# ad3002/aindex

Measured on AMD Instinct MI355X. Metric: kmer_lookups_per_sec_23mer_batch, higher is better.
Workload: dtype u64

## Files before the change

### aindex_amd/_lib.py

```python
from __future__ import annotations

import ctypes as C
import os
import re
import subprocess

_HERE = os.path.dirname(os.path.abspath(__file__))
ROOT = os.path.dirname(_HERE)
LIB_PATH = os.path.join(_HERE, "lib", "libaindex_hip.so")
CSRC = os.path.join(_HERE, "csrc")
HEADER = os.path.join(ROOT, "include", "aindex_hip.h")

AIX_OK = 0
AIX_ERR_CONFLICT = -12
AIX_ERR_ARG = -1
AIX_ERR_FORMAT = -3
AIX_ERR_NOMEM = -4
AIX_ERR_UNSUPPORTED = -6
AIX_ERR_MODE = -7
FMT_AUTO, FMT_PLAIN, FMT_FASTA, FMT_FASTQ = -1, 0, 1, 2
CANON_NONE, CANON_REF_X86, CANON_TRUE_RC = 0, 1, 2
TOTAL_13MERS = 4 ** 13
DIR_NEXT, DIR_PREV, DIR_BOTH = 0, 1, 2
WALK_GREEDY, WALK_UNITIG = 0, 1
# ... 27 lines not shown
                ("buckets", C.c_uint64), ("bucket_unfiled_keys", C.c_uint64), ("bucket_lanes", C.c_uint32), ("absence_filter_words", C.c_uint32),
                ("minimizer_lines", C.c_uint64), ("minimizer_unfiled_keys", C.c_uint64), ("count23_backend", C.c_uint32), ("count23_passes", C.c_uint32), ("positions_backend", C.c_uint32), ("reserved0", C.c_uint32),
                ("aindex_attached", C.c_uint32), ("ridx_on_device", C.c_uint32), ("aindex_entries", C.c_uint64), ("ridx_reads", C.c_uint64)]


class IngestStats(C.Structure):
    _fields_ = [("bytes_in", C.c_uint64), ("plain_bytes", C.c_uint64), ("parts", C.c_uint64), ("part_bytes", C.c_uint64), ("pieces", C.c_uint64),
                ("pinned_bytes", C.c_uint64), ("device_bytes", C.c_uint64), ("workspace_bytes", C.c_uint64), ("seconds_total", C.c_double), ("seconds_read", C.c_double),
                ("seconds_wait", C.c_double), ("seconds_h2d", C.c_double), ("seconds_normalise", C.c_double), ("seconds_compute", C.c_double), ("seconds_output", C.c_double)]

    def as_dict(self):
        return {n: getattr(self, n) for n, _ in self._fields_}


CONT_FIELDS = [("tf", "<u4", (4,)), ("n", "<u4"), ("sum", "<u4"), ("best_tf", "<u4"), ("best_base", "<u4")]


def cont_dtype():
    import numpy as np
    return np.dtype(CONT_FIELDS)


def readfix_dtype():
    import numpy as np
    return np.dtype(READFIX_FIELDS)


_LIB = None
vp, u64, u32, i32 = C.c_void_p, C.c_uint64, C.c_uint32, C.c_int

SIGNATURES = {
    "aix_version": (C.c_char_p, []),
    "aix_strerror": (C.c_char_p, [i32]),
    "aix_device_count": (i32, [C.POINTER(i32)]),
    "aix_pf_check": (i32, [vp, u64, C.POINTER(u64 * 4)]),
    "aix_index_open_23": (i32, [C.c_char_p, C.c_char_p, C.c_char_p, i32, C.POINTER(vp)]),
    "aix_index_open_13": (i32, [C.c_char_p, C.c_char_p, i32, C.POINTER(vp)]),
    "aix_index_create_23": (i32, [vp, u64, vp, vp, u64, i32, C.POINTER(vp)]),
    "aix_index_create_13": (i32, [vp, u64, vp, i32, C.POINTER(vp)]),
    "aix_index_close": (i32, [vp]),
    "aix_index_info": (i32, [vp, C.POINTER(Info)]),
    "aix_index_set_canonical_fastpath": (i32, [vp, i32]),
    "aix_index_set_fingerprint_filter": (i32, [vp, i32]),
    "aix_index_set_early_exit": (i32, [vp, i32]),
    "aix_index_set_bucket_table": (i32, [vp, i32, i32]),
    "aix_index_set_absence_filter": (i32, [vp, i32]),
    "aix_index_set_minimizer_table": (i32, [vp, i32]),
    "aix_index_set_tf_13": (i32, [vp, vp]),
    "aix_index_get_tf": (i32, [vp, vp, u64]),
    "aix_index_get_checker": (i32, [vp, vp, u64]),
    "aix_tf_batch_ascii": (i32, [vp, vp, u64, vp]),
    "aix_tf_batch_ascii_dev": (i32, [vp, vp, u64, vp, vp]),
    "aix_lookup_binned_stats": (i32, [vp, vp]),
    "aix_tf_batch_codes": (i32, [vp, vp, u64, vp]),
    "aix_tf_batch_codes_dev": (i32, [vp, vp, u64, vp, vp]),
    "aix_tf_batch_ragged": (i32, [vp, vp, vp, u64, vp]),
    "aix_tf_batch_ragged_dev": (i32, [vp, vp, vp, u64, vp, vp]),
    "aix_lines_batch_ascii_dev": (i32, [vp, vp, u64, vp, vp]),
    "aix_hash_batch_ascii": (i32, [vp, vp, u64, vp]),
    "aix_hash_batch_ascii_dev": (i32, [vp, vp, u64, vp, vp]),
    "aix_kid_strand_batch_ascii": (i32, [vp, vp, u64, vp, vp]),
    "aix_kid_strand_batch_ascii_dev": (i32, [vp, vp, u64, vp, vp, vp]),
    "aix_tf_both_batch_ascii": (i32, [vp, vp, u64, vp, vp]),
    "aix_tf_both_batch_ascii_dev": (i32, [vp, vp, u64, vp, vp, vp]),
    "aix_tf_total_batch_ascii": (i32, [vp, vp, u64, vp]),
    "aix_tf_total_batch_ascii_dev": (i32, [vp, vp, u64, vp, vp]),
    "aix_coverage_batch": (i32, [vp, vp, vp, u64, u32, vp, vp]),
    "aix_coverage_batch_dev": (i32, [vp, vp, vp, u64, u64, u32, vp, vp, vp]),
    "aix_count13": (i32, [vp, vp, u64, i32, vp]),
    "aix_count13_dev": (i32, [vp, vp, u64, vp, vp]),
    "aix_count23_fixed": (i32, [vp, vp, u64, i32, i32, vp]),
    "aix_count23_fixed_dev": (i32, [vp, vp, u64, i32, vp, vp]),
    "aix_ingest_warm": (i32, [i32]),
    "aix_count13_file": (i32, [vp, C.c_char_p, i32, C.c_char_p, vp, C.POINTER(IngestStats)]),
    "aix_count23_fixed_file": (i32, [vp, C.c_char_p, i32, i32, vp, C.POINTER(IngestStats)]),
    "aix_count_distinct_file": (i32, [C.c_char_p, i32, i32, i32, u64, i32, C.POINTER(vp), C.POINTER(vp), C.POINTER(u64), C.POINTER(IngestStats)]),
    "aix_merge_runs_dev": (i32, [vp, vp, vp, u32, u64, i32, vp, C.POINTER(vp)]),
    "aix_count_distinct": (i32, [vp, u64, i32, i32, i32, u64, i32, C.POINTER(vp), C.POINTER(vp), C.POINTER(u64)]),
    "aix_positions_fill": (i32, [vp, vp, u64, vp, vp, u64, C.POINTER(u64)]),
    "aix_positions_total": (i32, [vp, C.POINTER(u64)]),
    "aix_positions_fill_dev": (i32, [vp, vp, u64, u64, vp, vp, u64, vp]),
    "aix_positions_bucket_counts": (i32, [vp, vp, u64, i32, vp]),
    "aix_aindex_attach": (i32, [vp, vp, vp, u64]),
    "aix_aindex_attach_dev": (i32, [vp, vp, vp, u64, vp]),
    "aix_aindex_detach": (i32, [vp]),
    "aix_ridx_sorted_disjoint": (i32, [vp, u64]),
    "aix_ridx_attach": (i32, [vp, vp, u64]),
    "aix_positions_query": (i32, [vp, vp, u64, u64, C.POINTER(vp), C.POINTER(vp), C.POINTER(vp), C.POINTER(vp)]),
    "aix_positions_query_dev": (i32, [vp, vp, u64, u64, vp, vp, vp, vp, u64, C.POINTER(u64), vp]),
    "aix_positions_locate": (i32, [vp, vp, u64, vp, vp]),
    "aix_positions_locate_dev": (i32, [vp, vp, u64, vp, vp, vp]),
    "aix_reads_attach": (i32, [vp, vp, u64]),
    "aix_reads_attach_dev": (i32, [vp, vp, u64, vp]),
    "aix_reads_detach": (i32, [vp]),
    "aix_reads_info": (i32, [vp, C.POINTER(u64 * 2)]),
    "aix_reads_fetch": (i32, [vp, vp, vp, vp, u64, C.POINTER(vp), C.POINTER(vp)]),
    "aix_reads_fetch_dev": (i32, [vp, vp, vp, vp, u64, vp, vp, u64, C.POINTER(u64), vp]),
    "aix_reads_fetch_rid": (i32, [vp, vp, u64, C.POINTER(vp), C.POINTER(vp)]),
    "aix_reads_fetch_rid_dev": (i32, [vp, vp, u64, vp, vp, u64, C.POINTER(u64), vp]),
    "aix_reads_by_kmers": (i32, [vp, vp, u64, u64, C.POINTER(vp), C.POINTER(vp), C.POINTER(vp), C.POINTER(vp)]),
    "aix_reads_by_kmers_dev": (i32, [vp, vp, u64, u64, vp, vp, vp, u64, vp, u64, C.POINTER(u64 * 2), vp]),
    "aix_neighbours": (i32, [vp, vp, vp, u64, i32, u32, vp]),
    "aix_neighbours_dev": (i32, [vp, vp, vp, u64, i32, u32, vp, vp]),
    "aix_walk": (i32, [vp, vp, vp, u64, i32, u64, u32, i32, vp, vp, vp, vp, vp]),
    "aix_walk_dev": (i32, [vp, vp, vp, u64, i32, u64, u32, i32, vp, vp, vp, vp, vp, vp]),
    "aix_unitigs_layout_dev": (i32, [vp, u32, vp, vp, vp, C.POINTER(u64), C.POINTER(u64), C.POINTER(u64), C.POINTER(u64), vp]),
# ... 144 lines not shown
```

### aindex_amd/csrc/aix_device.hpp

```cpp
#pragma once
#include <hip/hip_runtime.h>
#include <stdint.h>

#define AIX_HD __host__ __device__ __forceinline__

namespace aix {

struct __attribute__((aligned(16))) BvRec {
    uint32_t pairs;
    uint32_t prefix;
    uint64_t fp;
};
struct __attribute__((aligned(32))) EeRec {
    uint32_t pairs;
    uint32_t prefix;
    uint32_t mask[6];
};
struct __attribute__((aligned(16))) KeyRec {
    uint64_t code;
    uint32_t tf;
    uint32_t pad;
};

struct __attribute__((aligned(16))) BkEntry {
    uint32_t code_lo;
    uint32_t code_hi;
    uint32_t tf;
    uint32_t slot;
};
#define AIX_BK_HI_MASK 0x3FFFFFFFu
#define AIX_BK_OVERFLOW 0x80000000u
#define AIX_BK_EMPTY_HI 0x3FFFFFFFu
#define AIX_BK_NONE 0xFFFFFFFFu

AIX_HD uint32_t rot32(uint32_t x, uint32_t k) { return (x << k) | (x >> (32u - k)); }
AIX_HD void filter_key(uint64_t code, uint32_t& hw, uint32_t& hb) {
    uint32_t a = (uint32_t)code + 0x9E3779B9u, b = (uint32_t)(code >> 32) + 0x85EBCA6Bu, c = 0xC2B2AE35u;
    c ^= b; c -= rot32(b, 14);
    a ^= c; a -= rot32(c, 11);
    b ^= a; b -= rot32(a, 25);
    c ^= b; c -= rot32(b, 16);
    a ^= c; a -= rot32(c, 4);
    b ^= a; b -= rot32(a, 14);
    c ^= b; c -= rot32(b, 24);
    hw = b;
    hb = c;
}
AIX_HD uint64_t bloom_mask(uint32_t hb) {
    const uint32_t lo = (1u << (hb & 15)) | (0x10000u << ((hb >> 4) & 15)), hi = (1u << ((hb >> 8) & 15)) | (0x10000u << ((hb >> 12) & 15));
    return (uint64_t)lo | ((uint64_t)hi << 32);
}
AIX_HD uint32_t bloom_word(uint32_t hw, uint32_t nwords) { return (uint32_t)(((uint64_t)hw * nwords) >> 32); }

struct FastMod {
    uint64_t d;
    uint32_t dn;
    uint32_t v;
    uint32_t s;
    uint32_t wide;
};

inline FastMod make_fastmod(uint64_t d) {
    FastMod f{};
    f.d = d;
    if (d == 0) { f.wide = 1; f.d = 1; return f; }
    if (d >> 32) { f.wide = 1; return f; }
    uint32_t d32 = (uint32_t)d;
    f.s = (uint32_t)__builtin_clz(d32);
    f.dn = d32 << f.s;
    f.v = (uint32_t)((~0ull) / f.dn - (1ull << 32));
    return f;
}

AIX_HD uint32_t rem_2by1(uint32_t u1, uint32_t u0, uint32_t d, uint32_t v) {
    uint64_t q = (uint64_t)v * u1 + (((uint64_t)u1 << 32) | u0);
    uint32_t q1 = (uint32_t)(q >> 32) + 1u, q0 = (uint32_t)q;
    uint32_t r = u0 - q1 * d;
    if (r > q0) r += d;
    if (r >= d) r -= d;
    return r;
}

AIX_HD uint64_t fastmod(uint64_t h, const FastMod& f) {
    if (f.wide) return h % f.d;
    const uint32_t s = f.s;
    const uint32_t hi = (uint32_t)(h >> 32), lo = (uint32_t)h;
    const uint32_t u2 = s ? (hi >> (32 - s)) : 0u;
    const uint32_t u1 = s ? ((hi << s) | (lo >> (32 - s))) : hi;
    const uint32_t u0 = lo << s;
    uint32_t r = rem_2by1(u2, u1, f.dn, f.v);
    r = rem_2by1(r, u0, f.dn, f.v);
    return (uint64_t)(r >> s);
}

AIX_HD void jmix(uint64_t& a, uint64_t& b, uint64_t& c) {
    a -= b; a -= c; a ^= (c >> 43);
    b -= c; b -= a; b ^= (a << 9);
    c -= a; c -= b; c ^= (b >> 8);
    a -= b; a -= c; a ^= (c >> 38);
    b -= c; b -= a; b ^= (a << 23);
    c -= a; c -= b; c ^= (b >> 5);
    a -= b; a -= c; a ^= (c >> 35);
    b -= c; b -= a; b ^= (a << 49);
    c -= a; c -= b; c ^= (b >> 11);
// ... 452 lines not shown
```

### aindex_amd/csrc/aix_handle.hpp

```cpp
#pragma once
#include <hip/hip_runtime.h>

#include <mutex>
#include <string>

#include "../../include/aindex_hip.h"
#include "aix_internal.hpp"

using namespace aix;

void set_last_error(const std::string& s);

#define HIPCHK(expr)                                                                          \
    do {                                                                                      \
        hipError_t _e = (expr);                                                               \
        if (_e != hipSuccess) {                                                               \
            set_last_error(std::string(#expr) + ": " + hipGetErrorString(_e));                \
            return AIX_ERR_HIP;                                                               \
        }                                                                                     \
    } while (0)


struct DevGuard {
    int prev = -1;
// ... 15 lines not shown
    bool pooled = true;
    hipError_t alloc(uint64_t bytes) { return pool_alloc(&p, bytes ? bytes : 1); }
    hipError_t alloc_once(uint64_t bytes) { pooled = false; return hipMalloc(&p, bytes ? bytes : 1); }
    ~DevBuf() { if (p) { (void)hipStreamSynchronize(st); if (pooled) pool_free(p); else (void)hipFree(p); } }
};

struct aix_index {
    int device = 0;
    uint32_t k = 0;
    uint64_t n = 0;
    uint64_t mphf_n = 0, D = 0, seed = 0, B = 0, W = 0;
    BvRec* recs = nullptr;
    EeRec* ee = nullptr;
    KeyRec* keys = nullptr;
    uint32_t* side = nullptr;
    KeyRec* unfiled = nullptr;
    uint64_t n_unfiled = 0;
    BkEntry* bk = nullptr;
    uint32_t nb = 0;
    bool bk_borrowed = false;
    uint32_t bk_lpp = 8;
    bool bk_lpp_set = false;
    uint64_t bk_unfiled = 0;
    bool bk_enabled = true;
    BkEntry* mk = nullptr;
    uint32_t* mk_off = nullptr;
    uint32_t mk_cap = 16;
    uint32_t nbm = 0;
    uint64_t mk_unfiled = 0;
    bool mk_enabled = true;
    uint64_t* bloom = nullptr;
    uint32_t nbloom = 0;
    bool bloom_enabled = true;
    uint64_t* tf13_mphf = nullptr;
    uint64_t* tf13_code = nullptr;
    uint32_t* perm13 = nullptr;
    unsigned long long* scratch13 = nullptr;
    void* count_ws = nullptr;
    uint64_t count_ws_bytes = 0;
    void* pin_in = nullptr;
    void* pin_out[3] = {nullptr, nullptr, nullptr};
    std::mutex small_mutex;
    hipStream_t small_stream = nullptr;
    void* pin_cov = nullptr;
    struct HostPipe* pipe = nullptr;
    std::mutex pipe_mutex;
    hipEvent_t count_done = nullptr;
    hipStream_t hist_stream = nullptr;
    hipStream_t probe_stream = nullptr;
    hipEvent_t probe_ev[2] = {nullptr, nullptr}, hist_ev[2] = {nullptr, nullptr}, start_ev = nullptr;
    void* lb_ws = nullptr;
    uint64_t lb_ws_bytes = 0;
    uint64_t* lb_stats = nullptr;
    hipEvent_t lb_done = nullptr;
    hipStream_t lb_stream = nullptr;
    bool lb_used = false;
    std::mutex lb_mutex;
    uint64_t device_bytes = 0;
    bool perm13_bijective = false;
    bool canonical_only = false;
    bool canonical_fastpath = true;
    bool has_fp = false;
    bool fp_filter = true;
    bool early_exit = true;
    std::mutex count_mutex;
    uint64_t pos_total = 0;
    bool pos_total_known = false;
    uint32_t a2_backend = 0;
    uint32_t c23_backend = 0, c23_passes = 0;
    bool c13_atomics = false, c13_added = false;
    uint64_t* ai_indices = nullptr;
    uint64_t* ai_positions = nullptr;
    uint64_t ai_total = 0;
    bool ai_attached = false, ai_owned = false;
    uint64_t* rx = nullptr;
    uint64_t rx_n = 0;
    bool rx_attached = false;
    uint8_t* rd = nullptr;
    uint64_t rd_len = 0;
    bool rd_attached = false, rd_owned = false;

    IndexDev dev_slots() const {
        IndexDev d = dev();
        if (!bk_lpp_set) d.bk_lpp = 2;
        return d;
    }
    IndexDev dev() const {
        IndexDev d{};
        d.m.recs = recs;
        d.m.ee = ee;
        d.m.D = D;
        d.m.seed = seed;
        d.m.nrecs = (B + 15) / 16;
        d.m.fm = make_fastmod(D);
        d.keys = keys;
        d.side = side;
        d.bk_store = bk;
        d.unfiled = unfiled;
        d.n = n;
        d.tf13_code = tf13_code;
        d.tf13_mphf = tf13_mphf;
        d.perm13 = perm13;
        d.canonical_only = (canonical_only && canonical_fastpath) ? 1u : 0u;
        d.k = k;
        d.use_fp = (has_fp && fp_filter) ? 1u : 0u;
        d.early_exit = (has_fp && ee && early_exit) ? 1u : 0u;
// ... 33 lines not shown
```

### aindex_amd/csrc/aix_lookup_binned.hip

```cpp
#include <algorithm>

#include "aix_env.hpp"
#include "aix_handle.hpp"

namespace aix {

static constexpr int LB_TB = 512;
static constexpr int LB_QPL = 8;
static constexpr int LB_TILE = LB_TB * LB_QPL;
static constexpr int LB_CH = 256;
static constexpr int LB_LINE = 16;
static constexpr int LB_MAXBINS = 256;
static_assert(LB_CH % LB_LINE == 0 && LB_LINE <= 64, "lines do not straddle chunks; one wave instruction moves a carry");
static constexpr unsigned LB_GRID_A = 768;
static constexpr int LB_FB = 512;
static constexpr int LB_CPG = LB_FB / LB_CH;
static constexpr int LB_U = 2;
static constexpr int LB_CPT = LB_U * LB_CPG;
static constexpr int LB_TICKETS = 8;
static constexpr int LB_SURV = 4096;
static constexpr int LB_FLUSH_AT = LB_SURV - LB_U * LB_FB;
static constexpr unsigned LB_GRID_B = 1024;
static_assert(LB_FB % LB_CH == 0 && LB_FB >= LB_MAXBINS && LB_FB % 64 == 0, "pass B scans the slices' chunk counts with one lane per slice");
static_assert(LB_FLUSH_AT > 0, "LB_SURV holds the flush threshold plus one trip's records");
static constexpr uint32_t LB_SAMPLES = 16384;
static constexpr uint32_t LB_IDX_BITS = 27, LB_WORD_BITS = 18, LB_MASK_BITS = 16;
static_assert(LB_MASK_BITS == 16 && LB_IDX_BITS + LB_WORD_BITS + LB_MASK_BITS <= 64, "the record holds the 16 bits bloom_mask reads");
static constexpr uint32_t LB_NONE = 0xFFFFFFFFu;
static constexpr uint32_t LB_LO_BITS = 32 - LB_IDX_BITS, LB_META_LO = 9;
static_assert(LB_IDX_BITS < 32 && LB_MAXBINS < (1 << LB_META_LO) && LB_META_LO + LB_LO_BITS <= 16 && LB_TILE <= (1 << 13), "that word never equals LB_NONE");
static constexpr uint64_t LB_HDR_BYTES = 4096;
enum { LB_FLAG = 0, LB_PASSED = 1, LB_DONE = 2, LB_NSURV = 3, LB_CURSOR = 16, LB_TICKET = 512 };

static constexpr uint32_t LB_NO_SHIFT = 32;
struct LbGeom {
    uint32_t nbins;
    uint32_t wps;
    uint32_t inv;
    uint32_t shift;
    uint32_t cap;
};
struct LbWs {
    uint32_t* hdr;
    uint32_t* list;
    uint32_t* cnt;
    uint64_t* rec;
    unsigned long long* stats;
};

__device__ __forceinline__ bool lb_hash(uint64_t w0, uint64_t w1, uint64_t w2, uint32_t& hw, uint32_t& hb) {
    uint64_t code;
    if (!encode23_clean(w0, w1, w2, code)) return false;
    const uint64_t r = revcomp(code, 23);
    filter_key(code <= r ? code : r, hw, hb);
    return true;
}

__device__ __forceinline__ void lb_slice(uint32_t word, const LbGeom& g, uint32_t& bin, uint32_t& wi) {
    if (g.shift != LB_NO_SHIFT) {
        bin = word >> g.shift;
        wi = word & (g.wps - 1);
    } else {
        bin = __umulhi(word, g.inv);
        wi = word - bin * g.wps;
        if (wi >= g.wps) { wi -= g.wps; ++bin; }
    }
}

__global__ void __launch_bounds__(256) k_lb_gate(const uint64_t* __restrict__ bloom, uint32_t nbloom, const uint8_t* __restrict__ q, uint32_t n,
                                                 uint32_t nsamp, int force, uint32_t* __restrict__ hdr, unsigned long long* __restrict__ stats) {
    if (force) {
        if (blockIdx.x == 0 && threadIdx.x == 0) { hdr[LB_FLAG] = 1u; atomicAdd(&stats[0], 1ull); }
        return;
    }
    __shared__ uint32_t s_pass;
    if (threadIdx.x == 0) s_pass = 0;
    __syncthreads();
    const uint32_t s = blockIdx.x * 256 + threadIdx.x;
    bool pass = false;
    if (s < nsamp) {
        const uint64_t i = (uint64_t)s * n / nsamp;
        uint64_t w0, w1, w2;
        uint32_t hw, hb;
        load23(q + 23 * i, w0, w1, w2);
// ... 228 lines not shown
        __syncthreads();
        for (uint32_t i = t; i < s_n; i += LB_FB) w.list[s_base + i] = surv[i];
        __syncthreads();
        if (t == 0) s_n = 0;
        __syncthreads();
    };
    const uint32_t nt = min(gridDim.x, (uint32_t)LB_TICKETS);
    const uint32_t lane_x = blockIdx.x % nt;
    uint32_t* const ticket = w.hdr + LB_TICKET + 32 * lane_x;
    uint32_t bin = 0;
    for (;;) {
        if (t == 0) s_ticket = atomicAdd(ticket, 1u);
        __syncthreads();
        const uint64_t it64 = ((uint64_t)s_ticket * nt + lane_x) * LB_CPT;
        if (it64 >= total) break;
        const uint32_t it = (uint32_t)it64;
        uint64_t r[LB_U], wd[LB_U];
        uint32_t cn[LB_U], wbase[LB_U];
#pragma unroll
        for (int u = 0; u < LB_U; ++u) {
            const uint32_t item = it + u * LB_CPG + t / LB_CH;
            cn[u] = 0; r[u] = 0; wbase[u] = 0;
            if (item < total) {
                while (bin + 1 < NB && item >= pre[bin + 1]) ++bin;
                const uint64_t ch = (uint64_t)bin * g.cap + (item - pre[bin]);
                cn[u] = w.cnt[ch];
                r[u] = __builtin_nontemporal_load(&w.rec[ch * LB_CH + t % LB_CH]);
                wbase[u] = bin * g.wps;
            }
        }
#pragma unroll
        for (int u = 0; u < LB_U; ++u) {
            const uint32_t word = wbase[u] + ((uint32_t)(r[u] >> LB_IDX_BITS) & ((1u << LB_WORD_BITS) - 1));
            wd[u] = (t % LB_CH < cn[u] && word < nbloom) ? bloom[word] : 0ull;
        }
#pragma unroll
        for (int u = 0; u < LB_U; ++u) {
            const uint64_t mk = bloom_mask((uint32_t)(r[u] >> (LB_IDX_BITS + LB_WORD_BITS)));
            const bool pass = t % LB_CH < cn[u] && (wd[u] & mk) == mk;
            const uint64_t m = __ballot(pass);
            if (m) {
                uint32_t r0 = 0;
                if ((t & 63u) == 0) r0 = atomicAdd(&s_n, (uint32_t)__popcll(m));
                r0 = __shfl(r0, 0);
                if (pass) surv[r0 + (uint32_t)__popcll(m & ((1ull << (t & 63u)) - 1))] = (uint32_t)r[u] & ((1u << LB_IDX_BITS) - 1);
            }
        }
        __syncthreads();
        if (s_n > (uint32_t)LB_FLUSH_AT) flush();
    }
    if (s_n) flush();
}

}

static uint64_t align_up(uint64_t x, uint64_t a) { return (x + a - 1) / a * a; }

void lookup_binned_release(aix_index* h) {
    if (h->lb_done) { (void)hipEventSynchronize(h->lb_done); (void)hipEventDestroy(h->lb_done); h->lb_done = nullptr; }
    if (h->lb_ws) { (void)hipFree(h->lb_ws); h->lb_ws = nullptr; h->lb_ws_bytes = 0; }
    if (h->lb_stats) { (void)hipFree(h->lb_stats); h->lb_stats = nullptr; }
}

int lookup23_binned(aix_index* h, const IndexDev& d, const uint8_t* q, uint64_t N, uint32_t* out, hipStream_t s) {
    const long sw = env_int("AIX_LOOKUP_BINNED", 0, 2, 1);
    if (sw == 0 || d.k != 23 || !d.canonical_only || !d.bk || !d.bloom || d.nbloom == 0) return AIX_LB_NOT_TAKEN;
    if (sw == 1 && N < env_u64("AIX_LOOKUP_BINNED_MIN", 0, ~0ull, AIX_LB_DEFAULT_MIN)) return AIX_LB_NOT_TAKEN;
    const uint64_t slice_bytes = env_u64("AIX_LOOKUP_SLICE_BYTES", 8, 2ull << 20, 1ull << 20);
    LbGeom g;
    g.wps = (uint32_t)std::min<uint64_t>(std::max<uint64_t>(slice_bytes / 8, 1), d.nbloom);
    g.nbins = (d.nbloom + g.wps - 1) / g.wps;
    if (g.nbins > (uint32_t)LB_MAXBINS) return AIX_LB_NOT_TAKEN;
    g.inv = g.wps > 1 ? (uint32_t)((1ull << 32) / g.wps) : 0xFFFFFFFFu;
    g.shift = (g.wps & (g.wps - 1)) == 0 ? (uint32_t)__builtin_ctz(g.wps) : LB_NO_SHIFT;
    const uint64_t piece = std::min<uint64_t>(std::min<uint64_t>(N, 1ull << LB_IDX_BITS), env_u64("AIX_LOOKUP_PIECE", 1, 1ull << LB_IDX_BITS, 1ull << LB_IDX_BITS));
    const uint64_t test_grid_a = env_u64("AIX_LOOKUP_TEST_GRID_A", 1, LB_GRID_A, LB_GRID_A);
    const unsigned grid_a = (unsigned)std::min<uint64_t>((piece + LB_TILE - 1) / LB_TILE, test_grid_a);
    const uint32_t carry_bytes = g.nbins * LB_LINE * 8;
    const uint64_t test_cap = env_u64("AIX_LOOKUP_TEST_BIN_CAP", 0, ~0ull, ~0ull);
    uint64_t cap = test_cap != ~0ull ? (test_cap + LB_CH - 1) / LB_CH : (piece + piece / 4) / g.nbins / LB_CH + 2 + grid_a;
    cap = std::min<uint64_t>(cap, (piece + LB_CH - 1) / LB_CH + grid_a);
    g.cap = (uint32_t)cap;
    const uint64_t off_list = LB_HDR_BYTES, off_cnt = align_up(off_list + 4 * piece, 256), off_rec = align_up(off_cnt + 4ull * g.nbins * cap, 256);
    const uint64_t need = off_rec + 8ull * g.nbins * cap * LB_CH;

    std::lock_guard<std::mutex> lk(h->lb_mutex);
    if (!h->lb_done && hipEventCreateWithFlags(&h->lb_done, hipEventDisableTiming) != hipSuccess) { (void)hipGetLastError(); h->lb_done = nullptr; return AIX_LB_NOT_TAKEN; }
    if (!h->lb_stats) {
        if (hipMalloc((void**)&h->lb_stats, 32) != hipSuccess) { (void)hipGetLastError(); h->lb_stats = nullptr; return AIX_LB_NOT_TAKEN; }
        HIPCHK(hipMemset(h->lb_stats, 0, 32));
    }
    if (need > h->lb_ws_bytes) {
        if (h->lb_used) HIPCHK(hipEventSynchronize(h->lb_done));
        if (h->lb_ws) { (void)hipFree(h->lb_ws); h->lb_ws = nullptr; h->lb_ws_bytes = 0; }
        if (hipMalloc(&h->lb_ws, need) != hipSuccess) { (void)hipGetLastError(); h->lb_ws = nullptr; return AIX_LB_NOT_TAKEN; }
        h->lb_ws_bytes = need;
    }
    if (h->lb_used && h->lb_stream != s) HIPCHK(hipStreamWaitEvent(s, h->lb_done, 0));
    h->lb_used = true;
    h->lb_stream = s;
    struct RecordOnExit {
        hipEvent_t ev; hipStream_t s;
        ~RecordOnExit() { (void)hipEventRecord(ev, s); }
    } record_on_exit{h->lb_done, s};

    if (carry_bytes > (16u << 10)) HIPCHK(hipFuncSetAttribute((const void*)k_lb_bin, hipFuncAttributeMaxDynamicSharedMemorySize, (int)carry_bytes));
    uint8_t* const base = (uint8_t*)h->lb_ws;
    LbWs w;
    w.hdr = (uint32_t*)base;
    w.list = (uint32_t*)(base + off_list);
    w.cnt = (uint32_t*)(base + off_cnt);
    w.rec = (uint64_t*)(base + off_rec);
    w.stats = (unsigned long long*)h->lb_stats;
    const uint64_t test_grid_b = env_u64("AIX_LOOKUP_TEST_GRID_B", 1, LB_GRID_B, LB_GRID_B);
    const unsigned grid_b = (unsigned)std::min<uint64_t>(std::max<uint64_t>(((uint64_t)g.nbins * cap + LB_CPT - 1) / LB_CPT, 1), test_grid_b);
    for (uint64_t lo = 0; lo < N; lo += piece) {
        const uint32_t m = (uint32_t)std::min<uint64_t>(piece, N - lo);
        const uint8_t* qp = q + 23 * lo;
        uint32_t* op = out + lo;
        HIPCHK(hipMemsetAsync(w.hdr, 0, LB_HDR_BYTES, s));
        const uint32_t nsamp = std::min<uint32_t>(m, LB_SAMPLES);
        hipLaunchKernelGGL(k_lb_gate, dim3(sw == 2 ? 1 : (nsamp + 255) / 256), dim3(256), 0, s, d.bloom, d.nbloom, qp, m, nsamp, sw == 2 ? 1 : 0, w.hdr,
                           w.stats);
        HIPCHK(hipGetLastError());
        if (sw != 2) HIPCHK(launch_lookup23_ascii(d, qp, m, MODE_TF, LookupOut{op, nullptr, nullptr, nullptr}, s, w.hdr + LB_FLAG));
        hipLaunchKernelGGL(k_lb_bin, dim3(std::min<unsigned>(grid_a, (m + LB_TILE - 1) / LB_TILE)), dim3(LB_TB), carry_bytes, s, d.nbloom, qp, m, g, w, op);
        HIPCHK(hipGetLastError());
        hipLaunchKernelGGL(k_lb_filter, dim3(grid_b), dim3(LB_FB), 0, s, d.bloom, d.nbloom, g, w);
        HIPCHK(hipGetLastError());
        HIPCHK(launch_lookup23_list(d, qp, w.list, w.hdr + LB_NSURV, m, w.hdr + LB_FLAG, op, w.stats + 3, s));
    }
    return AIX_LB_TAKEN;
}

extern "C" int aix_lookup_binned_stats(aix_index_t* h, uint64_t out[4]) {
    if (!h || !out) return AIX_ERR_ARG;
    DevGuard g(h->device);
    std::lock_guard<std::mutex> lk(h->lb_mutex);
    for (int i = 0; i < 4; ++i) out[i] = 0;
    if (!h->lb_stats) return AIX_OK;
    if (h->lb_used) HIPCHK(hipEventSynchronize(h->lb_done));
    HIPCHK(hipMemcpy(out, h->lb_stats, 32, hipMemcpyDeviceToHost));
    return AIX_OK;
}
```

### include/aindex_hip.h

```cpp
#ifndef AINDEX_HIP_H
#define AINDEX_HIP_H

#include <stddef.h>
#include <stdint.h>

#ifdef __cplusplus
extern "C" {
#endif

#define AIX_OK               0
#define AIX_ERR_ARG         -1
#define AIX_ERR_IO          -2
#define AIX_ERR_FORMAT      -3
#define AIX_ERR_NOMEM       -4
#define AIX_ERR_HIP         -5
#define AIX_ERR_UNSUPPORTED -6
#define AIX_ERR_MODE        -7
#define AIX_ERR_CONFLICT   -12

#define AIX_TOTAL_13MERS 67108864ull

#define AIX_FMT_AUTO  -1
#define AIX_FMT_PLAIN  0
#define AIX_FMT_FASTA  1
// ... 21 lines not shown
    uint32_t bucket_lanes;
    uint32_t absence_filter_words;
    uint64_t minimizer_lines;
    uint64_t minimizer_unfiled_keys;
    uint32_t count23_backend;
    uint32_t count23_passes;
    uint32_t positions_backend;
    uint32_t reserved0;
    uint32_t aindex_attached;
    uint32_t ridx_on_device;
    uint64_t aindex_entries;
    uint64_t ridx_reads;
} aix_info_t;

const char* aix_version(void);
const char* aix_strerror(int status);
int aix_device_count(int* count);
void aix_scratch_trim(void);
int aix_host_alloc(uint64_t bytes, void** out);
int aix_host_free(void* p);

int aix_pf_check(const void* pf_bytes, uint64_t pf_len, uint64_t hdr_out[4]);
int aix_index_open_23(const char* pf_path, const char* tf_bin_path, const char* kmers_bin_path,
                      int device, aix_index_t** out);
int aix_index_open_13(const char* pf_path, const char* tf_bin_path ,
                      int device, aix_index_t** out);
int aix_index_create_23(const void* pf_bytes, uint64_t pf_len, const uint64_t* checker,
                        const uint32_t* tf, uint64_t n, int device, aix_index_t** out);
int aix_index_create_13(const void* pf_bytes, uint64_t pf_len, const uint64_t* tf ,
                        int device, aix_index_t** out);
int aix_index_close(aix_index_t* h);
int aix_index_info(const aix_index_t* h, aix_info_t* info);
int aix_index_set_canonical_fastpath(aix_index_t* h, int enabled);
int aix_index_set_fingerprint_filter(aix_index_t* h, int enabled);
int aix_index_set_early_exit(aix_index_t* h, int enabled);
int aix_index_set_bucket_table(aix_index_t* h, int enabled, int lanes);
int aix_index_set_absence_filter(aix_index_t* h, int enabled);
int aix_index_set_minimizer_table(aix_index_t* h, int enabled);
int aix_index_set_tf_13(aix_index_t* h, const uint64_t* tf);
int aix_index_get_tf(const aix_index_t* h, void* out, uint64_t out_bytes);
int aix_index_get_checker(const aix_index_t* h, uint64_t* out, uint64_t n);

int aix_index_scatter(const void* pf_bytes, uint64_t pf_len, const char* keys, const uint32_t* counts, uint64_t n,
                      int device, uint64_t* checker_out, uint32_t* tf_out);
int aix_index_scatter_shard(const void* pf_bytes, uint64_t pf_len, const char* keys, const uint32_t* counts, uint64_t n_keys,
                            uint64_t n_slots, int device, uint64_t* checker_out, uint32_t* tf_out, uint32_t* occupied_out);
int aix_index_build_23_codes_dev(const void* pf_bytes, uint64_t pf_len, const uint64_t* d_codes,
                                 const uint32_t* d_counts , uint64_t n, int device, void* stream,
                                 aix_index_t** out);

int aix_tf_batch_ascii(aix_index_t* h, const char* kmers, uint64_t N, uint32_t* out);
int aix_tf_batch_ascii_dev(aix_index_t* h, const char* d_kmers, uint64_t N, uint32_t* d_out, void* stream);
int aix_lookup_binned_stats(aix_index_t* h, uint64_t out[4]);
int aix_tf_batch_codes(aix_index_t* h, const uint64_t* codes, uint64_t N, uint32_t* out);
int aix_tf_batch_codes_dev(aix_index_t* h, const uint64_t* d_codes, uint64_t N, uint32_t* d_out, void* stream);
int aix_tf_batch_ragged(aix_index_t* h, const char* bytes, const uint64_t* offsets, uint64_t N, uint32_t* out);
int aix_tf_batch_ragged_dev(aix_index_t* h, const char* d_bytes, const uint64_t* d_offsets, uint64_t N,
                            uint32_t* d_out, void* stream);

int aix_lines_batch_ascii_dev(aix_index_t* h, const char* d_kmers, uint64_t N, uint32_t* d_out, void* stream);
int aix_hash_batch_ascii(aix_index_t* h, const char* kmers, uint64_t N, uint64_t* out);
int aix_hash_batch_ascii_dev(aix_index_t* h, const char* d_kmers, uint64_t N, uint64_t* d_out, void* stream);
int aix_kid_strand_batch_ascii(aix_index_t* h, const char* kmers, uint64_t N, uint64_t* kid_out ,
                               uint8_t* strand_out );
int aix_kid_strand_batch_ascii_dev(aix_index_t* h, const char* d_kmers, uint64_t N, uint64_t* d_kid,
                                   uint8_t* d_strand, void* stream);
int aix_tf_both_batch_ascii(aix_index_t* h, const char* kmers, uint64_t N, uint64_t* fwd_out, uint64_t* rc_out);
int aix_tf_both_batch_ascii_dev(aix_index_t* h, const char* d_kmers, uint64_t N, uint64_t* d_fwd,
                                uint64_t* d_rc, void* stream);
int aix_tf_total_batch_ascii(aix_index_t* h, const char* kmers, uint64_t N, uint64_t* out);
int aix_tf_total_batch_ascii_dev(aix_index_t* h, const char* d_kmers, uint64_t N, uint64_t* d_out, void* stream);

int aix_coverage_batch(aix_index_t* h, const char* seqs, const uint64_t* offs, uint64_t M, uint32_t cutoff,
                       uint32_t* out, const uint64_t* out_offs);
int aix_coverage_batch_dev(aix_index_t* h, const char* d_seqs, const uint64_t* d_offs, uint64_t M,
                           uint64_t total_bytes, uint32_t cutoff, uint32_t* d_out, const uint64_t* d_out_offs,
                           void* stream);

int aix_count13(aix_index_t* h, const char* buf, uint64_t len, int format, uint64_t* tf_out);
int aix_count13_dev(aix_index_t* h, const char* d_plain, uint64_t len, uint64_t* d_tf_out, void* stream);
int aix_count23_fixed(aix_index_t* h, const char* buf, uint64_t len, int format, int canon_mode, uint32_t* tf_out);
int aix_count23_fixed_dev(aix_index_t* h, const char* d_plain, uint64_t len, int canon_mode,
                          uint32_t* d_tf_out , void* stream);
typedef struct {
    uint64_t bytes_in;
    uint64_t plain_bytes;
    uint64_t parts;
    uint64_t part_bytes;
    uint64_t pieces;
    uint64_t pinned_bytes;
    uint64_t device_bytes;
    uint64_t workspace_bytes;
    double seconds_total;
    double seconds_read;
    double seconds_wait;
    double seconds_h2d;
    double seconds_normalise;
    double seconds_compute;
    double seconds_output;
} aix_ingest_stats_t;
int aix_ingest_warm(int device);
int aix_count13_file(aix_index_t* h, const char* path, int format, const char* out_path , uint64_t* tf_out ,
                     aix_ingest_stats_t* stats);
int aix_count23_fixed_file(aix_index_t* h, const char* path, int format, int canon_mode, uint32_t* tf_out , aix_ingest_stats_t* stats);
int aix_window_codes_dev(const char* d_plain, uint64_t len, int k, int canon_mode, uint64_t* d_codes, void* stream);
int aix_positions_fill(aix_index_t* h, const char* reads, uint64_t len, uint64_t* indices_out, uint64_t* positions_out,
// ... 325 lines not shown
```

Baseline: 75.43 billion.

## Add coarse folded-bloom prefilter held in LDS for binned lookup filter pass

Builds a per-bin byte image that folds each 64-bit bloom word into 8 bits and caches it across calls, keyed on the bloom pointer and geometry. A new filter kernel loads a bin's image into LDS and tests each record against it first. Only records that pass fetch the full bloom word from global memory, which is meant to cut random global traffic for absent k-mers. In exchange it adds a fold kernel on first use, extra memory, a larger LDS footprint, and a different grid and unroll shape. It is enabled by default when the bin's word count fits.

```diff
diff --git a/aindex_amd/_lib.py b/aindex_amd/_lib.py
--- a/aindex_amd/_lib.py
+++ b/aindex_amd/_lib.py
@@ -103,6 +103,7 @@
     "aix_tf_batch_ascii": (i32, [vp, vp, u64, vp]),
     "aix_tf_batch_ascii_dev": (i32, [vp, vp, u64, vp, vp]),
     "aix_lookup_binned_stats": (i32, [vp, vp]),
+    "aix_lookup_binned_coarse_stats": (i32, [vp, vp]),
     "aix_tf_batch_codes": (i32, [vp, vp, u64, vp]),
     "aix_tf_batch_codes_dev": (i32, [vp, vp, u64, vp, vp]),
     "aix_tf_batch_ragged": (i32, [vp, vp, vp, u64, vp]),
diff --git a/aindex_amd/csrc/aix_device.hpp b/aindex_amd/csrc/aix_device.hpp
--- a/aindex_amd/csrc/aix_device.hpp
+++ b/aindex_amd/csrc/aix_device.hpp
@@ -50,6 +50,11 @@
     const uint32_t lo = (1u << (hb & 15)) | (0x10000u << ((hb >> 4) & 15)), hi = (1u << ((hb >> 8) & 15)) | (0x10000u << ((hb >> 12) & 15));
     return (uint64_t)lo | ((uint64_t)hi << 32);
 }
+AIX_HD uint32_t bloom_fold(uint64_t word) {
+    const uint32_t q0 = (uint32_t)word & 0xFFFFu;
+    return (q0 & 0xFFu) | (q0 >> 8);
+}
+AIX_HD bool bloom_fold_test(uint32_t folded, uint32_t hb) { return ((folded >> (hb & 7u)) & 1u) != 0; }
 AIX_HD uint32_t bloom_word(uint32_t hw, uint32_t nwords) { return (uint32_t)(((uint64_t)hw * nwords) >> 32); }
 
 struct FastMod {
diff --git a/aindex_amd/csrc/aix_handle.hpp b/aindex_amd/csrc/aix_handle.hpp
--- a/aindex_amd/csrc/aix_handle.hpp
+++ b/aindex_amd/csrc/aix_handle.hpp
@@ -91,6 +91,10 @@
     void* lb_ws = nullptr;
     uint64_t lb_ws_bytes = 0;
     uint64_t* lb_stats = nullptr;
+    uint8_t* lb_coarse = nullptr;
+    uint64_t lb_coarse_bytes = 0;
+    const uint64_t* lb_coarse_src = nullptr;
+    uint32_t lb_coarse_nbloom = 0, lb_coarse_wps = 0;
     hipEvent_t lb_done = nullptr;
     hipStream_t lb_stream = nullptr;
     bool lb_used = false;
diff --git a/aindex_amd/csrc/aix_lookup_binned.hip b/aindex_amd/csrc/aix_lookup_binned.hip
--- a/aindex_amd/csrc/aix_lookup_binned.hip
+++ b/aindex_amd/csrc/aix_lookup_binned.hip
@@ -23,6 +23,16 @@
 static constexpr unsigned LB_GRID_B = 1024;
 static_assert(LB_FB % LB_CH == 0 && LB_FB >= LB_MAXBINS && LB_FB % 64 == 0, "pass B scans the slices' chunk counts with one lane per slice");
 static_assert(LB_FLUSH_AT > 0, "LB_SURV holds the flush threshold plus one trip's records");
+static constexpr int LBC_FB = 1024;
+static constexpr int LBC_CPG = LBC_FB / LB_CH;
+static constexpr int LBC_U = 4;
+static constexpr int LBC_CPT = LBC_U * LBC_CPG;
+static constexpr int LBC_SURV = 6144;
+static constexpr int LBC_FLUSH_AT = LBC_SURV - LBC_U * LBC_FB;
+static constexpr unsigned LBC_GRID = 256;
+static constexpr uint32_t LBC_MAX_WPS = 1u << 17;
+static_assert(LBC_FB % LB_CH == 0 && LBC_FB >= LB_MAXBINS && LBC_FLUSH_AT > 0, "as for pass B without the image");
+static_assert(LBC_MAX_WPS + 4 * (LBC_SURV + 2 * LB_MAXBINS + 1 + LBC_FB / 64 + 5) <= 160u << 10, "image, survivors and tables fit the LDS of a CU");
 static constexpr uint32_t LB_SAMPLES = 16384;
 static constexpr uint32_t LB_IDX_BITS = 27, LB_WORD_BITS = 18, LB_MASK_BITS = 16;
 static_assert(LB_MASK_BITS == 16 && LB_IDX_BITS + LB_WORD_BITS + LB_MASK_BITS <= 64, "the record holds the 16 bits bloom_mask reads");
@@ -30,6 +40,7 @@
 static constexpr uint32_t LB_LO_BITS = 32 - LB_IDX_BITS, LB_META_LO = 9;
 static_assert(LB_IDX_BITS < 32 && LB_MAXBINS < (1 << LB_META_LO) && LB_META_LO + LB_LO_BITS <= 16 && LB_TILE <= (1 << 13), "that word never equals LB_NONE");
 static constexpr uint64_t LB_HDR_BYTES = 4096;
+static constexpr int LB_NSTATS = 6;
 enum { LB_FLAG = 0, LB_PASSED = 1, LB_DONE = 2, LB_NSURV = 3, LB_CURSOR = 16, LB_TICKET = 512 };
 
 static constexpr uint32_t LB_NO_SHIFT = 32;
@@ -364,6 +375,120 @@
     if (s_n) flush();
 }
 
+__global__ void __launch_bounds__(256) k_lb_fold(const uint64_t* __restrict__ bloom, uint32_t nbloom, uint32_t wps, uint32_t stride, uint32_t nbins,
+                                                 uint8_t* __restrict__ coarse) {
+    const uint32_t total = nbins * stride;
+    for (uint32_t i = blockIdx.x * 256 + threadIdx.x; i < total; i += gridDim.x * 256) {
+        const uint32_t s = i / stride, wi = i - s * stride;
+        const uint64_t word = (uint64_t)s * wps + wi;
+        coarse[i] = (wi < wps && word < nbloom) ? (uint8_t)bloom_fold(bloom[word]) : (uint8_t)0;
+    }
+}
+
+__global__ void __launch_bounds__(LBC_FB) k_lb_filter_coarse(const uint64_t* __restrict__ bloom, uint32_t nbloom, const uint8_t* __restrict__ coarse,
+                                                             uint32_t stride, LbGeom g, LbWs w) {
+    if (!w.hdr[LB_FLAG]) return;
+    extern __shared__ __attribute__((aligned(16))) uint8_t image[];
+    __shared__ uint32_t tpre[LB_MAXBINS + 1];
+    __shared__ uint32_t nch[LB_MAXBINS];
+    __shared__ uint32_t surv[LBC_SURV];
+    __shared__ uint32_t wsum[LBC_FB / 64];
+    __shared__ uint32_t s_n, s_base, s_ticket, s_cnt[2];
+    const uint32_t t = threadIdx.x, NB = g.nbins;
+    const uint32_t nt = min(gridDim.x, (uint32_t)LB_TICKETS);
+    const uint32_t lane_x = blockIdx.x % nt;
+    uint32_t* const ticket = w.hdr + LB_TICKET + 32 * lane_x;
+    const uint32_t mine = t < NB ? min(w.hdr[LB_CURSOR + t], g.cap) : 0u;
+    uint32_t total;
+    const uint32_t excl = lb_scan_excl<LBC_FB>(t % nt == lane_x ? (mine + LBC_CPT - 1) / LBC_CPT : 0u, wsum, total);
+    if (t < (uint32_t)LB_MAXBINS) { tpre[t] = excl; nch[t] = mine; }
+    if (t == 0) { tpre[LB_MAXBINS] = total; s_n = 0; s_cnt[0] = 0; s_cnt[1] = 0; }
+    __syncthreads();
+    auto flush = [&]() {
+        if (t == 0) s_base = atomicAdd(&w.hdr[LB_NSURV], s_n);
+        __syncthreads();
+        for (uint32_t i = t; i < s_n; i += LBC_FB) w.list[s_base + i] = surv[i];
+        __syncthreads();
+        if (t == 0) s_n = 0;
+        __syncthreads();
+    };
+    uint32_t bin = 0;
+    auto locate = [&](uint32_t k, uint32_t& c0) -> bool {
+        if (k >= total) return false;
+        while (k >= tpre[bin + 1]) ++bin;
+        c0 = (k - tpre[bin]) * LBC_CPT;
+        return true;
+    };
+    auto fetch = [&](uint32_t b, uint32_t c0, bool live, uint64_t (&r)[LBC_U], uint32_t (&cn)[LBC_U]) {
+        const uint32_t last = nch[b] - 1;
+#pragma unroll
+        for (int u = 0; u < LBC_U; ++u) {
+            const uint32_t ci = c0 + u * LBC_CPG + t / LB_CH;
+            const uint64_t ch = (uint64_t)b * g.cap + min(ci, last);
+            const uint32_t c = w.cnt[ch];
+            r[u] = __builtin_nontemporal_load(&w.rec[ch * LB_CH + t % LB_CH]);
+            cn[u] = live && ci <= last ? c : 0u;
+        }
+    };
+    uint64_t rn[LBC_U];
+    uint32_t cnn[LBC_U], bn, c0 = 0;
+    if (t == 0) s_ticket = atomicAdd(ticket, 1u);
+    __syncthreads();
+    bool more = locate(s_ticket, c0);
+    bn = bin;
+    if (more) fetch(bn, c0, true, rn, cnn);
+    __syncthreads();
+    uint32_t held = LB_NONE, n_tested = 0, n_on = 0;
+    while (more) {
+        uint64_t r[LBC_U], wd[LBC_U];
+        uint32_t cn[LBC_U];
+        bool on[LBC_U];
+        const uint32_t b = bn;
+#pragma unroll
+        for (int u = 0; u < LBC_U; ++u) { r[u] = rn[u]; cn[u] = cnn[u]; }
+        if (t == 0) s_ticket = atomicAdd(ticket, 1u);
+        if (b != held) {
+            const uint4* const src = (const uint4*)(coarse + (uint64_t)b * stride);
+            for (uint32_t i = t; i < stride / 16; i += LBC_FB) ((uint4*)image)[i] = src[i];
+            held = b;
+        }
+        __syncthreads();
+#pragma unroll
+        for (int u = 0; u < LBC_U; ++u) {
+            const uint32_t wi = (uint32_t)(r[u] >> LB_IDX_BITS) & ((1u << LB_WORD_BITS) - 1), word = b * g.wps + wi;
+            const bool valid = t % LB_CH < cn[u] && wi < g.wps && word < nbloom;
+            on[u] = valid && bloom_fold_test(image[valid ? wi : 0u], (uint32_t)(r[u] >> (LB_IDX_BITS + LB_WORD_BITS)));
+            wd[u] = bloom[on[u] ? word : b * g.wps];
+            n_tested += (uint32_t)__popcll(__ballot(valid));
+            n_on += (uint32_t)__popcll(__ballot(on[u]));
+        }
+#pragma unroll
+        for (int u = 0; u < LBC_U; ++u) {
+            const uint64_t mk = bloom_mask((uint32_t)(r[u] >> (LB_IDX_BITS + LB_WORD_BITS)));
+            const bool pass = on[u] && (wd[u] & mk) == mk;
+            const uint64_t m = __ballot(pass);
+            if (m) {
+                uint32_t r0 = 0;
+                if ((t & 63u) == 0) r0 = atomicAdd(&s_n, (uint32_t)__popcll(m));
+                r0 = __shfl(r0, 0);
+                if (pass) surv[r0 + (uint32_t)__popcll(m & ((1ull << (t & 63u)) - 1))] = (uint32_t)r[u] & ((1u << LB_IDX_BITS) - 1);
+            }
+        }
+        more = locate(s_ticket, c0);
+        bn = bin;
+        fetch(bn, more ? c0 : 0u, more, rn, cnn);
+        __syncthreads();
+        if (s_n > (uint32_t)LBC_FLUSH_AT) flush();
+    }
+    if ((t & 63u) == 0 && n_tested) { atomicAdd(&s_cnt[0], n_tested); atomicAdd(&s_cnt[1], n_on); }
+    if (s_n) flush();
+    __syncthreads();
+    if (t == 0 && s_cnt[0]) {
+        atomicAdd(&w.stats[4], (unsigned long long)s_cnt[0]);
+        atomicAdd(&w.stats[5], (unsigned long long)s_cnt[1]);
+    }
+}
+
 }
 
 static uint64_t align_up(uint64_t x, uint64_t a) { return (x + a - 1) / a * a; }
@@ -372,6 +497,7 @@
     if (h->lb_done) { (void)hipEventSynchronize(h->lb_done); (void)hipEventDestroy(h->lb_done); h->lb_done = nullptr; }
     if (h->lb_ws) { (void)hipFree(h->lb_ws); h->lb_ws = nullptr; h->lb_ws_bytes = 0; }
     if (h->lb_stats) { (void)hipFree(h->lb_stats); h->lb_stats = nullptr; }
+    if (h->lb_coarse) { (void)hipFree(h->lb_coarse); h->lb_coarse = nullptr; h->lb_coarse_bytes = 0; h->lb_coarse_src = nullptr; }
 }
 
 int lookup23_binned(aix_index* h, const IndexDev& d, const uint8_t* q, uint64_t N, uint32_t* out, hipStream_t s) {
@@ -395,12 +521,24 @@
     g.cap = (uint32_t)cap;
     const uint64_t off_list = LB_HDR_BYTES, off_cnt = align_up(off_list + 4 * piece, 256), off_rec = align_up(off_cnt + 4ull * g.nbins * cap, 256);
     const uint64_t need = off_rec + 8ull * g.nbins * cap * LB_CH;
+    const uint64_t coarse_max = std::min<uint64_t>(env_u64("AIX_LOOKUP_TEST_COARSE_MAX", 0, LBC_MAX_WPS, LBC_MAX_WPS), LBC_MAX_WPS);
+    bool coarse = env_int("AIX_LOOKUP_COARSE", 0, 1, 1) == 1 && g.wps <= coarse_max;
+    const uint32_t cstride = (uint32_t)align_up(g.wps, 16);
+    const uint64_t need_coarse = (uint64_t)g.nbins * cstride;
 
     std::lock_guard<std::mutex> lk(h->lb_mutex);
     if (!h->lb_done && hipEventCreateWithFlags(&h->lb_done, hipEventDisableTiming) != hipSuccess) { (void)hipGetLastError(); h->lb_done = nullptr; return AIX_LB_NOT_TAKEN; }
     if (!h->lb_stats) {
-        if (hipMalloc((void**)&h->lb_stats, 32) != hipSuccess) { (void)hipGetLastError(); h->lb_stats = nullptr; return AIX_LB_NOT_TAKEN; }
-        HIPCHK(hipMemset(h->lb_stats, 0, 32));
+        if (hipMalloc((void**)&h->lb_stats, 8 * LB_NSTATS) != hipSuccess) { (void)hipGetLastError(); h->lb_stats = nullptr; return AIX_LB_NOT_TAKEN; }
+        HIPCHK(hipMemset(h->lb_stats, 0, 8 * LB_NSTATS));
+    }
+    if (coarse && need_coarse > h->lb_coarse_bytes) {
+        if (h->lb_used) HIPCHK(hipEventSynchronize(h->lb_done));
+        if (h->lb_coarse) { (void)hipFree(h->lb_coarse); h->lb_coarse = nullptr; }
+        h->lb_coarse_bytes = 0;
+        h->lb_coarse_src = nullptr;
+        if (hipMalloc((void**)&h->lb_coarse, need_coarse) != hipSuccess) { (void)hipGetLastError(); h->lb_coarse = nullptr; coarse = false; }
+        else h->lb_coarse_bytes = need_coarse;
     }
     if (need > h->lb_ws_bytes) {
         if (h->lb_used) HIPCHK(hipEventSynchronize(h->lb_done));
@@ -426,6 +564,18 @@
     w.stats = (unsigned long long*)h->lb_stats;
     const uint64_t test_grid_b = env_u64("AIX_LOOKUP_TEST_GRID_B", 1, LB_GRID_B, LB_GRID_B);
     const unsigned grid_b = (unsigned)std::min<uint64_t>(std::max<uint64_t>(((uint64_t)g.nbins * cap + LB_CPT - 1) / LB_CPT, 1), test_grid_b);
+    const unsigned grid_c = (unsigned)std::min<uint64_t>(std::max<uint64_t>((uint64_t)g.nbins * ((cap + LBC_CPT - 1) / LBC_CPT), 1), std::min<uint64_t>(test_grid_b, LBC_GRID));
+    if (coarse) {
+        if (h->lb_coarse_src != d.bloom || h->lb_coarse_nbloom != d.nbloom || h->lb_coarse_wps != g.wps) {
+            hipLaunchKernelGGL(k_lb_fold, dim3((unsigned)std::min<uint64_t>((need_coarse + 255) / 256, 4096)), dim3(256), 0, s, d.bloom, d.nbloom, g.wps, cstride,
+                               g.nbins, h->lb_coarse);
+            HIPCHK(hipGetLastError());
+            h->lb_coarse_src = d.bloom;
+            h->lb_coarse_nbloom = d.nbloom;
+            h->lb_coarse_wps = g.wps;
+        }
+        if (cstride > (16u << 10)) HIPCHK(hipFuncSetAttribute((const void*)k_lb_filter_coarse, hipFuncAttributeMaxDynamicSharedMemorySize, (int)cstride));
+    }
     for (uint64_t lo = 0; lo < N; lo += piece) {
         const uint32_t m = (uint32_t)std::min<uint64_t>(piece, N - lo);
         const uint8_t* qp = q + 23 * lo;
@@ -438,7 +588,8 @@
         if (sw != 2) HIPCHK(launch_lookup23_ascii(d, qp, m, MODE_TF, LookupOut{op, nullptr, nullptr, nullptr}, s, w.hdr + LB_FLAG));
         hipLaunchKernelGGL(k_lb_bin, dim3(std::min<unsigned>(grid_a, (m + LB_TILE - 1) / LB_TILE)), dim3(LB_TB), carry_bytes, s, d.nbloom, qp, m, g, w, op);
         HIPCHK(hipGetLastError());
-        hipLaunchKernelGGL(k_lb_filter, dim3(grid_b), dim3(LB_FB), 0, s, d.bloom, d.nbloom, g, w);
+        if (coarse) hipLaunchKernelGGL(k_lb_filter_coarse, dim3(grid_c), dim3(LBC_FB), cstride, s, d.bloom, d.nbloom, (const uint8_t*)h->lb_coarse, cstride, g, w);
+        else hipLaunchKernelGGL(k_lb_filter, dim3(grid_b), dim3(LB_FB), 0, s, d.bloom, d.nbloom, g, w);
         HIPCHK(hipGetLastError());
         HIPCHK(launch_lookup23_list(d, qp, w.list, w.hdr + LB_NSURV, m, w.hdr + LB_FLAG, op, w.stats + 3, s));
     }
@@ -455,3 +606,14 @@
     HIPCHK(hipMemcpy(out, h->lb_stats, 32, hipMemcpyDeviceToHost));
     return AIX_OK;
 }
+
+extern "C" int aix_lookup_binned_coarse_stats(aix_index_t* h, uint64_t out[2]) {
+    if (!h || !out) return AIX_ERR_ARG;
+    DevGuard g(h->device);
+    std::lock_guard<std::mutex> lk(h->lb_mutex);
+    out[0] = out[1] = 0;
+    if (!h->lb_stats) return AIX_OK;
+    if (h->lb_used) HIPCHK(hipEventSynchronize(h->lb_done));
+    HIPCHK(hipMemcpy(out, h->lb_stats + 4, 16, hipMemcpyDeviceToHost));
+    return AIX_OK;
+}
diff --git a/include/aindex_hip.h b/include/aindex_hip.h
--- a/include/aindex_hip.h
+++ b/include/aindex_hip.h
@@ -97,6 +97,7 @@
 int aix_tf_batch_ascii(aix_index_t* h, const char* kmers, uint64_t N, uint32_t* out);
 int aix_tf_batch_ascii_dev(aix_index_t* h, const char* d_kmers, uint64_t N, uint32_t* d_out, void* stream);
 int aix_lookup_binned_stats(aix_index_t* h, uint64_t out[4]);
+int aix_lookup_binned_coarse_stats(aix_index_t* h, uint64_t out[2]);
 int aix_tf_batch_codes(aix_index_t* h, const uint64_t* codes, uint64_t N, uint32_t* out);
 int aix_tf_batch_codes_dev(aix_index_t* h, const uint64_t* d_codes, uint64_t N, uint32_t* d_out, void* stream);
 int aix_tf_batch_ragged(aix_index_t* h, const char* bytes, const uint64_t* offsets, uint64_t N, uint32_t* out);
```

Result: faster. 89.01 billion (median of 6 runs) (+18.0%).
